# ZhangT-tech/MoCA-Video

Hardware: AMD Instinct MI355X
Metric: denoising UNet-steps/sec @16x320x512 fp16 (higher is better)
Workload: dtype f16

## Files before the change

### include/moca_hip.h

```cpp
#ifndef MOCA_HIP_H
#define MOCA_HIP_H

#include <stdint.h>

#ifdef __cplusplus
extern "C" {
#endif

#define MOCA_OK            0
#define MOCA_E_BADARG     -1
#define MOCA_E_LAUNCH     -2
#define MOCA_E_NODEVICE   -3
#define MOCA_E_GRAPH      -4

#define MOCA_A_LINEAR   0
#define MOCA_A_CONV3X3  1
#define MOCA_A_TCONV3   2

#define MOCA_EP_GEGLU   1
#define MOCA_EP_OUT_F32 2
#define MOCA_FORCE_SMALL_TILE 4
#define MOCA_EP_COLSUM 16
#define MOCA_EP_LN     32
#define MOCA_EP_GELU    8
// ... 24 lines not shown
    int32_t T;
    int32_t HW;
    int32_t flags;
    int32_t splits;
    int32_t nopad_lo;
    int32_t prefetch_kib;
    int32_t tattn_causal;
    float*      colsum;
    const float* ln_gamma;
    const float* ln_beta;
    void*       ln_out;
    int32_t     ld_ln;
    float       ln_eps;
    float*      rowsum;
    const float* lnf_part;
    const float* lnf_wsum;
    int32_t     lnf_nparts;
    int32_t     reserved2_;
    int64_t*    gstat;
    int32_t     gstat_rows;
    float       tattn_scale;
    const void* prefetch;
    int32_t     up_phase;
    int32_t     reserved4_;
    const void* a2;
    int32_t     lda2;
    int32_t     k1;
    int32_t     gstat_cpg;
    int32_t     gstat_coff;
    int32_t     wgroup_rows;
    int32_t     wgroup_stride;
} moca_gemm_params;

int moca_gemm_f16(const moca_gemm_params* p, void* stream);
int moca_gemm_colsum_rows(const moca_gemm_params* p);
int moca_gemm_ln_ok(const moca_gemm_params* p);
int moca_gemm_rowsum_cols(const moca_gemm_params* p);
int moca_gemm_lnfold_ok(const moca_gemm_params* p);
int moca_gemm_tattn_ok(const moca_gemm_params* p);
int moca_gemm_wgroup_ok(const moca_gemm_params* p);
int moca_gemm_cat_ok(const moca_gemm_params* p);
#define MOCA_ROUTE_SMALL64   1
#define MOCA_ROUTE_SMALL128  2
#define MOCA_ROUTE_GLDS128   3
#define MOCA_ROUTE_GLDS160   4
#define MOCA_ROUTE_G4        5
#define MOCA_ROUTE_W80       6
#define MOCA_ROUTE_W80W      7
#define MOCA_ROUTE_SQ256     8
#define MOCA_ROUTE_G4P       9
#define MOCA_ROUTE_SQP       10
#define MOCA_ROUTE_TATTN     11
#define MOCA_ROUTE_WS        12
int moca_gemm_route(const moca_gemm_params* p);
int moca_gemm_splitk_groupnorm_ok(const moca_gemm_params* p, int32_t HW, int32_t frames_per_stat);
int moca_gemm_splitk_groupnorm_f16(const moca_gemm_params* p, void* y, const float* gamma, const float* beta, int32_t HW,
                                   int32_t frames_per_stat, float eps, int32_t silu, int32_t write_x, void* stream);
int64_t moca_gemm_splitk_ws_bytes(int32_t M, int32_t N, int32_t splits);

int moca_groupnorm_nhwc_f16(const void* x, void* y, const float* gamma, const float* beta,
                            int32_t F, int32_t HW, int32_t C, int32_t frames_per_stat,
                            float eps, int32_t silu, float* ws, void* stream);
int64_t moca_groupnorm_ws_bytes(int32_t F, int32_t HW, int32_t C);
#define MOCA_GN_ROUTE_STREAM    1
#define MOCA_GN_ROUTE_SLAB2     2
#define MOCA_GN_ROUTE_SLAB4     3
#define MOCA_GN_ROUTE_SLAB8     4
#define MOCA_GN_ROUTE_SLABREG1  5
#define MOCA_GN_ROUTE_SLABREG2  6
#define MOCA_GN_ROUTE_SLABREG3  7
#define MOCA_GN_ROUTE_SLABREG4  8
int moca_groupnorm_route(int32_t F, int32_t HW, int32_t C, int32_t frames_per_stat);
int moca_groupnorm_nchunk(int32_t F, int32_t HW);
int moca_groupnorm_colsum_f16(const void* x, void* y, const float* gamma, const float* beta, const float* colsum,
                              int32_t tile_rows, int32_t F, int32_t HW, int32_t C, int32_t frames_per_stat,
                              float eps, int32_t silu, float* ws, void* stream);

int moca_groupnorm_fold_weights_f16(const void* w, const float* bias, const float* gamma, const float* beta, const int64_t* gstat,
                                    void* wg, float* bg, int32_t n_sg, int32_t N, int32_t K, int32_t ldw, int64_t count, float eps,
                                    void* stream);

int moca_groupnorm_gstat_f16(const void* x, void* y, const float* gamma, const float* beta, const int64_t* gstat,
                             int32_t F, int32_t HW, int32_t C, int32_t frames_per_stat,
                             float eps, int32_t silu, void* stream);
int moca_concat_channels_gstat_f16(const void* a, const void* b, void* out, int32_t F, int32_t HW, int32_t C1, int32_t C2,
                                   int32_t frames_per_stat, int64_t* gstat, void* stream);
int moca_groupnorm_gstat_cat_f16(const void* a, const void* b, void* y, const float* gamma, const float* beta,
                                 const int64_t* gstat_cat, const int64_t* gstat_b, int32_t Fb, int32_t F, int32_t HW, int32_t C1,
                                 int32_t C2, int32_t frames_per_stat, float eps, int32_t silu, void* stream);
int moca_gstat_accum_f16(const void* x, int32_t F, int32_t HW, int32_t C, int32_t frames_per_stat, int32_t cpg, int32_t coff,
                         int64_t* gstat, void* stream);
int moca_memset_zero(void* ptr, int64_t bytes, void* stream);

int moca_layernorm_f16(const void* x, void* y, const float* gamma, const float* beta,
                       int32_t M, int32_t C, float eps, void* stream);

int moca_attention_f16(const void* q, const void* k, const void* v, void* out,
                       int32_t Bq, int32_t heads, int32_t Nq, int32_t Nk,
                       int32_t ldq, int32_t ldk, int32_t ldv, int32_t ldo,
                       int32_t kv_div, float scale, void* stream);

int moca_attention_ip_f16(const void* q, const void* k, const void* v, const void* k_ip, const void* v_ip, void* out,
                          int32_t Bq, int32_t heads, int32_t Nq, int32_t Nt, int32_t Ni,
                          int32_t ldq, int32_t ldk, int32_t ldv, int32_t ldk_ip, int32_t ldv_ip, int32_t ldo,
                          int32_t kv_div, float scale, float ip_scale, void* stream);

// ... 95 lines not shown
    const int32_t* sam_idx;
    float cfg_scale, beta, one_minus_beta, gamma, one_minus_gamma;
    int32_t nW, C, Q, f, HW, wb_from;
} moca_fifo_step_params;
int moca_fifo_step_windows_f32(const moca_fifo_step_params* p, void* stream);
int moca_sam_select_masks_f32(const float* cand, const int32_t* cand_off, const int32_t* ncand, const int64_t* t_rows, float* eff,
                              int32_t* eff_idx, int32_t nW, int32_t f, int32_t HW, void* stream);
int moca_fifo_advance_f32(moca_fifo_state* state, float* queue, const float* newframe, float* emitted, int32_t n_slots,
                          int32_t emit_frame, float* mask, float* mask_sums, int32_t C, int32_t Q, int32_t HW, void* stream);
int moca_fifo_prepare_queue_f32(const float* z, const float* noise, float* queue, const float* coef_z, const float* coef_noise,
                                const int32_t* frame_idx, int32_t BC, int32_t Tz, int32_t Q, int32_t HW, void* stream);
int moca_base_set_timestep(const moca_fifo_state* state, const int64_t* table, int32_t S, int64_t* rows, int32_t n, void* stream);
int moca_base_ddim_step_f32(moca_fifo_state* state, float* x, const float* eps_c, const float* eps_u, const float* noise,
                            float* pred_x0, const float* coef, int32_t S, float cfg_scale, int32_t use_scale, int64_t n, void* stream);
#define MOCA_DDPM_X0 1
#define MOCA_DDPM_CLIP 2
#define MOCA_DDPM_SCALE 4
#define MOCA_DDPM_MASK_C0 8
int moca_ddpm_step_f32(moca_fifo_state* state, const float* x, float* out, const float* eps_c, const float* eps_u,
                       const float* noise, float* x_recon, float* mean, const float* mask, const float* x0,
                       const float* noise_q, const float* coef, const int64_t* t, int64_t t_stride, int32_t B, int32_t n_tab,
                       int64_t per, int64_t mask_inner, float cfg_scale, float temperature, int32_t flags, void* stream);
int moca_mask_frame_sums_f32(const float* mask, float* sums, int32_t frames, int32_t HW, void* stream);

int moca_freq_mix_3d_f32(const float* x, const float* noise, const float* lpf, float* out,
                         int32_t C, int32_t T, int32_t H, int32_t W, float* ws, void* stream);
int64_t moca_freq_mix_ws_bytes(int32_t C, int32_t T, int32_t H, int32_t W);
int moca_freq_filter_f32(float* lpf, int32_t T, int32_t H, int32_t W, int32_t type, int32_t n,
                         double d_s, double d_t, void* stream);

int moca_graph_begin(void* stream);
int moca_graph_end(void* stream, void** graph_exec_out);
int moca_graph_launch(void* graph_exec, void* stream);
int moca_graph_destroy(void* graph_exec);
int moca_stream_create(void** stream_out);
int moca_stream_destroy(void* stream);
int moca_stream_sync(void* stream);
int moca_event_create(void** ev_out);
int moca_event_record(void* ev, void* stream);
int moca_event_elapsed_ms(void* ev_start, void* ev_stop, float* ms_out);
int moca_event_destroy(void* ev);

#define MOCA_TUNE_GEMM_W80   0
#define MOCA_TUNE_GEMM_G4    1
#define MOCA_TUNE_GEMM_SQ256 2
#define MOCA_TUNE_GEMM_WIDE  3
#define MOCA_TUNE_GN_SLAB    4
#define MOCA_TUNE_GEMM_G4P   5
#define MOCA_TUNE_GEMM_MF32  6
#define MOCA_TUNE_GEMM_SQP   7
#define MOCA_TUNE_SQP_WALK   8
#define MOCA_TUNE_SLAB_F16   9
#define MOCA_TUNE_GEMM_WS    10
#define MOCA_TUNE_COUNT      11
int moca_set_tuning(int32_t knob, int32_t value);
int moca_debug_clock_sampler(void* buf, int32_t blocks, int32_t nsamples, const int32_t* stop, void* stream);

int moca_device_info(char* name, int32_t len, int32_t* cu_count);
const char* moca_version(void);

#ifdef __cplusplus
}
#endif
#endif
```

### moca_video_amd/csrc/gemm.hip

```cpp
#include "gemm_launch.h"

namespace {

template <int BN, int AMODE>
__global__ __launch_bounds__(256, 2) void gemm_f16_kernel(const moca_gemm_params p) {
    constexpr int NT = BN / 64;
    constexpr int B_SLOTS = BN / 32;
    constexpr int A_BYTES = BM * ROW_BYTES;
    constexpr int B_BYTES = BN * ROW_BYTES;

    extern __shared__ __attribute__((aligned(16))) char smem[];
    char* sA = smem;
    char* sB = smem + 2 * A_BYTES;

    const int tid = threadIdx.x, lane = tid & 63, wave = tid >> 6;
    const int wave_m = wave >> 1, wave_n = wave & 1;

    const int tiles_m = (p.M + BM - 1) / BM;
    const int tiles_n = p.N / BN;
    const int nblk = tiles_m * tiles_n * p.splits;
    int logical;
    remap_block<BN>(nblk, logical);
    const int split = logical % p.splits;
    const int tile = logical / p.splits;
// ... 369 lines not shown
            for (int j = 0; j < 8; ++j) { const float a = (float)v[i][j]; s += a; q += a * a; }
        }
    s = wave_sum(s); q = wave_sum(q);
    if ((tid & 63) == 0) { s_red[0][tid >> 6] = s; s_red[1][tid >> 6] = q; }
    __syncthreads();
    if (tid < cpg) {
        double a = 0.0, b = 0.0;
        for (int w = 0; w < (nthr >> 6); ++w) { a += (double)s_red[0][w]; b += (double)s_red[1][w]; }
        const double mean = a * inv_count;
        double var = b * inv_count - mean * mean;
        if (var < 0.0) var = 0.0;
        const float rstd = (float)(1.0 / sqrt(var + (double)eps));
        const float sc = rstd * gm_t;
        s_sc[tid] = sc;
        s_sh[tid] = bt_t - (float)mean * sc;
    }
    __syncthreads();
#pragma unroll
    for (int i = 0; i < CPT; ++i)
        if (mrow[i] >= 0) {
            const int c0 = ccol[i] - g * cpg;
            half8v r;
#pragma unroll
            for (int j = 0; j < 8; ++j) {
                float a = (float)v[i][j] * s_sc[c0 + j] + s_sh[c0 + j];
                if (silu) a = moca_silu(a);
                r[j] = (half_t)a;
            }
            *reinterpret_cast<half8v*>(y + (int64_t)mrow[i] * N + ccol[i]) = r;
        }
}

template <int BN, int AMODE>
int launch_gemm(const moca_gemm_params& p, hipStream_t st) {
    const int tiles_m = (p.M + BM - 1) / BM, tiles_n = p.N / BN;
    const int nblk = tiles_m * tiles_n * p.splits;
    constexpr int lds_pipe = 2 * (BM + BN) * ROW_BYTES;
    constexpr int lds_epi = BM * BN * 4;
    constexpr int lds = lds_pipe > lds_epi ? lds_pipe : lds_epi;
    if (!dyn_lds_once<&gemm_f16_kernel<BN, AMODE>>(lds)) return MOCA_E_LAUNCH;
    hipLaunchKernelGGL((gemm_f16_kernel<BN, AMODE>), dim3(nblk), dim3(256), lds, st, p);
    MOCA_CHECK_LAUNCH();
    return MOCA_OK;
}
int launch_gemm_small(int bn, const moca_gemm_params& p, hipStream_t st) {
    if (bn == 128) return with_gather(p, [&](auto am, auto) { return launch_gemm<128, decltype(am)::value>(p, st); });
    return with_gather(p, [&](auto am, auto) { return launch_gemm<64, decltype(am)::value>(p, st); });
}

enum Route : int {
    R_NONE = 0,
    R_SMALL64 = MOCA_ROUTE_SMALL64, R_SMALL128 = MOCA_ROUTE_SMALL128, R_GLDS128 = MOCA_ROUTE_GLDS128, R_GLDS160 = MOCA_ROUTE_GLDS160,
    R_G4 = MOCA_ROUTE_G4, R_W80 = MOCA_ROUTE_W80, R_W80W = MOCA_ROUTE_W80W, R_SQ256 = MOCA_ROUTE_SQ256, R_G4P = MOCA_ROUTE_G4P,
    R_SQP = MOCA_ROUTE_SQP, R_TATTN = MOCA_ROUTE_TATTN, R_WS = MOCA_ROUTE_WS,
};

void normalise_splits(moca_gemm_params& p) {
    if (p.splits < 1) p.splits = 1;
    if (p.splits > (p.K + BK - 1) / BK) p.splits = (p.K + BK - 1) / BK;
    if (p.splits > 1) {
        const int nkt = (p.K + BK - 1) / BK, kts = (nkt + p.splits - 1) / p.splits;
        p.splits = (nkt + kts - 1) / kts;
    }
}

inline int64_t a_span_bytes(const moca_gemm_params& p) {
    if (p.a_mode == MOCA_A_LINEAR) return ((int64_t)p.M * p.lda + 64) * 2;
    if (p.a_mode == MOCA_A_CONV3X3) return ((int64_t)(p.M / (p.outH * p.outW)) * p.inH * p.inW * p.C + 64) * 2;
    return ((int64_t)p.M * p.C + 64) * 2;
}
inline bool buffer_addressable(const moca_gemm_params& p) {
    if (p.a2 && ((int64_t)p.M * p.lda2 + 64) * 2 >= (1ll << 31)) return false;
    return a_span_bytes(p) < (1ll << 31) && (int64_t)p.N * p.ldw * 2 < (1ll << 31);
}

bool persistent_ok(const moca_gemm_params& p, int BN, int blocks) {
    if (p.a_mode != MOCA_A_LINEAR || p.splits != 1 || p.N % BN || p.K % 64 || !buffer_addressable(p)) return false;
    if (p.flags & ~(MOCA_EP_GEGLU | MOCA_EP_LNFOLD)) return false;
    if ((p.flags & MOCA_EP_GEGLU) && (p.residual || p.rowadd)) return false;
    return ((p.M + 255) / 256) * (p.N / BN) >= blocks;
}

Route route_of(const moca_gemm_params& p) {
    if (p.flags & MOCA_EP_TATTN) return R_TATTN;
    const int ws_mode = moca_tuning_get(MOCA_TUNE_GEMM_WS);
    if (ws_mode && moca_gemm_ws_ok(p) && (ws_mode == 2 || p.residual || p.M >= (1 << 17))) return R_WS;
    if (!p.a2 && p.wgroup_rows <= 0) {
        const int sqp_mode = moca_tuning_get(MOCA_TUNE_GEMM_SQP), g4p_mode = moca_tuning_get(MOCA_TUNE_GEMM_G4P);
        if (sqp_mode && persistent_ok(p, 256, SQP_BLOCKS) && (sqp_mode == 2 || (p.flags & MOCA_EP_GEGLU))) return R_SQP;
        if (g4p_mode && persistent_ok(p, 128, G4P_BLOCKS) && (g4p_mode == 2 || (p.flags & MOCA_EP_GEGLU))) return R_G4P;
    }
    const int w80_mode = moca_tuning_get(MOCA_TUNE_GEMM_W80);
    const int tiles320 = ((p.M + 319) / 320) * (p.N / 160);
    if (w80_mode && p.N % 160 == 0 && !(p.flags & (MOCA_EP_GEGLU | MOCA_EP_OUT_F32 | MOCA_FORCE_SMALL_TILE)) && p.M > 160 &&
        (tiles320 * p.splits >= 200 || w80_mode == 2) && fast_gather(p) && buffer_addressable(p)) {
        if (p.flags & MOCA_EP_LN) return R_W80W;
        const int wide_mode = moca_tuning_get(MOCA_TUNE_GEMM_WIDE);
        if (wide_mode == 0 || p.N % 320) return R_W80;
        return (p.a_mode == MOCA_A_LINEAR || wide_mode == 2) ? R_W80W : R_W80;
    }
    const int g4_mode = moca_tuning_get(MOCA_TUNE_GEMM_G4);
    const bool use_g4 = !(p.flags & MOCA_EP_OUT_F32) &&
                        (g4_mode == 2 || (g4_mode == 1 && (p.flags & MOCA_EP_GEGLU) && p.K <= 640 && p.M < (1 << 17)));
    const int sq256_mode = moca_tuning_get(MOCA_TUNE_GEMM_SQ256);
    if (sq256_mode && p.a_mode == MOCA_A_LINEAR && p.N % 256 == 0 && p.N >= 2560 && p.M >= 512 && fast_gather(p) && buffer_addressable(p) &&
        !(p.flags & (MOCA_EP_OUT_F32 | MOCA_FORCE_SMALL_TILE)) && ((p.M + 255) / 256) * (p.N / 256) * p.splits >= 200 &&
        (sq256_mode == 2 || !use_g4)) return R_SQ256;
    const int big_bn = (p.N % 128 == 0) ? 128 : (p.N % 160 == 0 ? 160 : 0);
    if (big_bn != 0 && p.M > 128 && !(p.flags & MOCA_FORCE_SMALL_TILE)) {
        if (big_bn == 128) return use_g4 ? R_G4 : R_GLDS128;
        return R_GLDS160;
    }
    return p.N % 128 == 0 ? R_SMALL128 : R_SMALL64;
}

constexpr int CAN_SPLITK = 1 << 16, CAN_A2 = 1 << 17, CAN_WGROUP = 1 << 18, CAN_UP_PHASE = 1 << 19;
constexpr int EP_STATS = MOCA_EP_COLSUM | MOCA_EP_GSTAT;
struct RouteInfo { int tm, tn, can; };
RouteInfo route_info(Route r) {
    constexpr int GLDS = MOCA_EP_GEGLU | MOCA_EP_OUT_F32 | EP_STATS | MOCA_EP_ROWSUM | MOCA_EP_LNFOLD | CAN_SPLITK | CAN_UP_PHASE;
    constexpr int W80 = EP_STATS | MOCA_EP_ROWSUM | MOCA_EP_LNFOLD | CAN_SPLITK | CAN_UP_PHASE | CAN_A2 | CAN_WGROUP;
    switch (r) {
        case R_SMALL64: return {BM, 64, MOCA_EP_OUT_F32 | MOCA_EP_GELU | CAN_SPLITK};
        case R_SMALL128: return {BM, 128, MOCA_EP_GEGLU | MOCA_EP_OUT_F32 | MOCA_EP_GELU | CAN_SPLITK};
        case R_GLDS128: return {256, 128, GLDS};
        case R_GLDS160: return {256, 160, GLDS};
        case R_G4: return {256, 128, MOCA_EP_GEGLU | MOCA_EP_LNFOLD | CAN_SPLITK | CAN_UP_PHASE};
        case R_W80: return {320, 160, W80};
        case R_W80W: return {160, 320, W80 | MOCA_EP_LN};
        case R_SQ256: return {256, 256, MOCA_EP_GEGLU | MOCA_EP_LNFOLD | CAN_SPLITK};
        case R_G4P: return {256, 128, MOCA_EP_GEGLU | MOCA_EP_LNFOLD};
        case R_SQP: return {256, 256, MOCA_EP_GEGLU | MOCA_EP_LNFOLD};
        case R_TATTN: return {320, 192, MOCA_EP_TATTN | MOCA_EP_LNFOLD};
        case R_WS: return {32, 80, MOCA_EP_ROWSUM | MOCA_EP_GSTAT | CAN_WGROUP};
        case R_NONE: break;
    }
    return {0, 0, 0};
}

bool route_can(Route r, const moca_gemm_params& p) {
    const RouteInfo ri = route_info(r);
    const int f = p.flags & ~(MOCA_FORCE_SMALL_TILE | MOCA_EP_SLABS);
    const int wants = f | (p.splits > 1 ? CAN_SPLITK : 0) | (p.a2 ? CAN_A2 : 0) | (p.wgroup_rows ? CAN_WGROUP : 0) | (p.up_phase ? CAN_UP_PHASE : 0);
    if (r == R_NONE || (wants & ~ri.can) || p.wgroup_rows < 0) return false;
    if (r == R_WS) return true;
    const bool linear1 = p.a_mode == MOCA_A_LINEAR && p.splits == 1;
    if (r == R_TATTN) {
        if (!linear1 || !fast_gather(p) || !buffer_addressable(p) || p.residual || p.rowadd || (p.flags & MOCA_FORCE_SMALL_TILE)) return false;
        if (p.N % 192 || p.T != 16 || p.HW <= 0 || p.HW % 20 || p.M % (16 * p.HW)) return false;
        if (p.ldo % 4 || p.ldo < p.N / 3) return false;
        return p.tattn_causal == 0 || (p.tattn_causal == 1 && p.tattn_scale > 0.f);
    }
    if ((f & EP_STATS) && (p.splits != 1 || (f & (MOCA_EP_GEGLU | MOCA_EP_OUT_F32)))) return false;
    if ((f & MOCA_EP_ROWSUM) && (p.splits != 1 || (f & (MOCA_EP_GEGLU | MOCA_EP_OUT_F32 | EP_STATS | MOCA_EP_LN | MOCA_EP_GELU)))) return false;
    if ((f & MOCA_EP_LN) && !(linear1 && p.N == 320 && !(f & EP_STATS))) return false;
    if ((f & MOCA_EP_LNFOLD) && !(linear1 && !(f & (MOCA_EP_OUT_F32 | EP_STATS | MOCA_EP_LN | MOCA_EP_ROWSUM | MOCA_EP_GELU)) &&
                                  !((r == R_GLDS128 || r == R_GLDS160) && (f & MOCA_EP_GEGLU)))) return false;
    if ((f & MOCA_EP_GELU) && (f & MOCA_EP_GEGLU)) return false;
    if (p.a2) {
        if (!linear1 || (f & ~(EP_STATS | MOCA_EP_ROWSUM))) return false;
        if (p.k1 <= 0 || p.k1 >= p.K || p.k1 % 64 || (p.K - p.k1) % 64 || p.lda % 8 || p.lda2 % 8 || p.lda < p.k1 || p.lda2 < p.K - p.k1) return false;
    }
    if (p.wgroup_rows) {
        if (!linear1 || p.a2 || p.wgroup_stride < p.N * p.ldw || (f & ~(EP_STATS | MOCA_EP_ROWSUM | MOCA_EP_LN))) return false;
        if (p.M % p.wgroup_rows || p.wgroup_rows % ri.tm) return false;
        if ((int64_t)(p.M / p.wgroup_rows) * p.wgroup_stride * 2 >= (1ll << 31)) return false;
    }
    if (p.up_phase && (p.splits != 1 || p.M <= 160 || !fast_gather(p) || p.residual || p.rowadd || (f & ~MOCA_EP_GSTAT) ||
                       (p.N % 128 && p.N % 160))) return false;
    return true;
}

Route checked_route(const moca_gemm_params& p) {
    const Route r = route_of(p);
    return route_can(r, p) ? r : R_NONE;
}

Route query_route(const moca_gemm_params* pp, int flag, moca_gemm_params& p) {
    if (!pp) return R_NONE;
    p = *pp;
    if (p.M <= 0 || p.N <= 0 || p.K <= 0 || p.N % 64 || p.K % 8) return R_NONE;
// ... 25 lines not shown
    if (p.splits > 1 && !p.splitk_ws) return R_NONE;
    if (p.prefetch_kib < 0 || (p.prefetch_kib > 0 && (!p.prefetch || (reinterpret_cast<uintptr_t>(p.prefetch) & 15)))) return R_NONE;
    if ((p.flags & MOCA_EP_GELU) && (p.splits != 1 || !((p.flags & MOCA_FORCE_SMALL_TILE) || p.M <= 128))) return R_NONE;
    normalise_splits(p);
    if ((p.flags & MOCA_EP_SLABS) && (p.splits < 2 || (p.flags & ~MOCA_EP_SLABS))) return R_NONE;
    if (p.up_phase && p.a_mode != MOCA_A_CONV3X3) return R_NONE;
    switch (p.a_mode) {
        case MOCA_A_LINEAR:
            if (!p.a2 && (p.lda % 8 || p.lda < p.K)) return R_NONE;
            break;
        case MOCA_A_CONV3X3:
            if (p.up_phase < 0 || p.up_phase > 4) return R_NONE;
            if (p.C % 8 || p.K != (p.up_phase ? 4 : 9) * p.C || p.inH <= 0 || p.inW <= 0 || p.outH <= 0 || p.outW <= 0) return R_NONE;
            if (p.up_phase && (p.stride != 1 || p.up || p.nopad_lo)) return R_NONE;
            if (p.stride != 1 && p.stride != 2) return R_NONE;
            if (p.nopad_lo != 0 && (p.nopad_lo != 1 || p.stride != 2 || p.up || (p.inH | p.inW) & 1)) return R_NONE;
            if (p.up && (p.stride != 1 || p.outH != 2 * p.inH || p.outW != 2 * p.inW)) return R_NONE;
            if (!p.up && p.stride == 1 && (p.outH != p.inH || p.outW != p.inW)) return R_NONE;
            if (p.stride == 2 && (p.outH != (p.inH - 1) / 2 + 1 || p.outW != (p.inW - 1) / 2 + 1)) return R_NONE;
            if (p.M % (p.outH * p.outW)) return R_NONE;
            break;
        case MOCA_A_TCONV3:
            if (p.C % 8 || p.K != 3 * p.C || p.T <= 0 || p.HW <= 0 || p.M % (p.T * p.HW)) return R_NONE;
            break;
        default:
            return R_NONE;
    }
    if (p.a2 && p.a_mode != MOCA_A_LINEAR) return R_NONE;
    if (p.gstat_cpg < 0 || p.gstat_coff < 0 || ((p.gstat_cpg || p.gstat_coff) && !(p.flags & MOCA_EP_GSTAT))) return R_NONE;
    if (p.tattn_causal && !(p.flags & MOCA_EP_TATTN)) return R_NONE;
    const Route r = checked_route(p);
    if (r == R_NONE) return R_NONE;
    if ((p.flags & MOCA_EP_COLSUM) && !p.colsum) return R_NONE;
    if ((p.flags & MOCA_EP_LN) && !(p.ln_gamma && p.ln_beta && p.ln_out && p.ld_ln % 8 == 0)) return R_NONE;
    if ((p.flags & MOCA_EP_ROWSUM) && !p.rowsum) return R_NONE;
    if ((p.flags & MOCA_EP_LNFOLD) && !(p.lnf_part && p.lnf_wsum && p.lnf_nparts >= 1)) return R_NONE;
    if ((p.flags & MOCA_EP_GSTAT) &&
        !(p.gstat && !(p.flags & MOCA_EP_COLSUM) && p.gstat_rows > 0 && p.gstat_rows % route_info(r).tm == 0 && p.M % p.gstat_rows == 0 &&
          (p.gstat_cpg > 0 ? (p.gstat_coff + p.N - 1) / p.gstat_cpg < 32 : (p.N % 32 == 0 && p.gstat_coff == 0)))) return R_NONE;
    p.reserved4_ = 0;
    if ((int64_t)p.M * (geglu ? p.N / 2 : p.N) * 2 >= (128ll << 20)) p.reserved4_ |= 1;
    if (slab_f16(r, p)) p.reserved4_ |= 4;
    return r;
}

int launch_route(Route r, const moca_gemm_params& p, hipStream_t st) {
    switch (r) {
        case R_TATTN: return moca_gemm_w80s_launch(3, p, st);
        case R_WS: return moca_gemm_ws_launch(p, st);
        case R_SQP: return moca_gemm_sqp_launch(p, st);
        case R_G4P: return moca_gemm_g4p_launch(p, st);
        case R_W80: return moca_gemm_w80s_launch(0, p, st);
        case R_W80W: return moca_gemm_w80s_launch(1, p, st);
        case R_SQ256: return moca_gemm_w80s_launch(2, p, st);
        case R_G4: return moca_gemm_g4_launch(p, st);
        case R_GLDS128: return moca_gemm_glds_launch(128, p, st);
        case R_GLDS160: return moca_gemm_glds_launch(160, p, st);
        case R_SMALL128: return launch_gemm_small(128, p, st);
        case R_SMALL64: return launch_gemm_small(64, p, st);
        case R_NONE: break;
    }
    return MOCA_E_BADARG;
}

}

#ifdef MOCA_STAMPS
extern "C" int moca_debug_stamps(unsigned long long* host_out, int n_blocks) {
    if (n_blocks > STAMP_BLOCKS) n_blocks = STAMP_BLOCKS;
    return hipMemcpyFromSymbol(host_out, HIP_SYMBOL(g_stamps), (size_t)n_blocks * STAMP_SLOTS * 8) == hipSuccess ? 0 : -2;
}
#endif

extern "C" int moca_gemm_route(const moca_gemm_params* pp) {
    moca_gemm_params p;
    return prepare(pp, p);
}

extern "C" int moca_gemm_colsum_rows(const moca_gemm_params* pp) {
    moca_gemm_params p;
    return route_info(query_route(pp, (pp && (pp->flags & MOCA_EP_GSTAT)) ? 0 : MOCA_EP_COLSUM, p)).tm;
}
extern "C" int moca_gemm_rowsum_cols(const moca_gemm_params* pp) {
    moca_gemm_params p;
    return route_info(query_route(pp, MOCA_EP_ROWSUM, p)).tn;
}
extern "C" int moca_gemm_ln_ok(const moca_gemm_params* pp) {
    moca_gemm_params p;
    return query_route(pp, MOCA_EP_LN, p) != R_NONE;
}
extern "C" int moca_gemm_lnfold_ok(const moca_gemm_params* pp) {
    moca_gemm_params p;
    return query_route(pp, MOCA_EP_LNFOLD, p) != R_NONE;
}
extern "C" int moca_gemm_tattn_ok(const moca_gemm_params* pp) {
    moca_gemm_params p;
    return query_route(pp, MOCA_EP_TATTN, p) != R_NONE;
}
extern "C" int moca_gemm_cat_ok(const moca_gemm_params* pp) {
    moca_gemm_params p;
    return query_route(pp, 0, p) != R_NONE && p.a2;
}
extern "C" int moca_gemm_wgroup_ok(const moca_gemm_params* pp) {
    moca_gemm_params p;
    return query_route(pp, 0, p) != R_NONE && p.wgroup_rows > 0;
}
// ... 58 lines not shown
```

### moca_video_amd/csrc/gemm_diag.hip

```cpp
#ifndef MOCA_DIAG_NAME
#error "gemm_diag.hip is the unit of the diagnostic builds: compile it with -DMOCA_DIAG_NAME"
#endif
#include "gemm.hip"
#include "gemm_tiled.hip"
#include "gemm_persistent.hip"
```

### moca_video_amd/csrc/gemm_launch.h

```cpp
#ifndef MOCA_GEMM_LAUNCH_H
#define MOCA_GEMM_LAUNCH_H
#include "gemm_device.h"

int moca_gemm_glds_launch(int bn, const moca_gemm_params& p, hipStream_t st);
int moca_gemm_g4_launch(const moca_gemm_params& p, hipStream_t st);
int moca_gemm_w80s_launch(int shape, const moca_gemm_params& p, hipStream_t st);
int moca_gemm_g4p_launch(const moca_gemm_params& p, hipStream_t st);
int moca_gemm_sqp_launch(const moca_gemm_params& p, hipStream_t st);

namespace {

constexpr int G4P_BLOCKS = 512;
constexpr int SQP_BLOCKS = 256;

static int choose_xcd_n(const moca_gemm_params& p, int tiles_m, int tiles_n, int BN) {
    if (p.splits != 1 || p.a_mode != MOCA_A_LINEAR) return 1;
    const double Wtot = (double)p.N * p.K * 2, Atot = (double)p.M * p.K * 2;
    auto cost = [&](int xn) {
        const int xm = 8 / xn;
        const double wsub = (double)(tiles_n / xn) * BN * p.K * 2;
        return (wsub <= 3.6e6 ? xm * Wtot : tiles_m * Wtot) + xn * Atot;
    };
    double best = cost(1);
    int best_xn = 1;
    for (int xn = 2; xn <= 8; xn *= 2) {
        if (tiles_m % (8 / xn) || tiles_n % xn) continue;
        const double c = cost(xn);
        if (c < 0.8 * best) { best = c; best_xn = xn; }
    }
    return best_xn;
}

inline bool fast_gather(const moca_gemm_params& p) {
    return (p.a_mode == MOCA_A_LINEAR) ? (p.K % BK == 0 && p.K <= 8192) : (p.C % BK == 0 && p.C <= 8192);
}
template <typename F>
int with_gather(const moca_gemm_params& p, F f) {
    const bool fast = fast_gather(p);
    if (p.a_mode == MOCA_A_LINEAR) return fast ? f(int_c<MOCA_A_LINEAR>{}, yes_t{}) : f(int_c<MOCA_A_LINEAR>{}, no_t{});
    if (p.a_mode == MOCA_A_CONV3X3) return fast ? f(int_c<MOCA_A_CONV3X3>{}, yes_t{}) : f(int_c<MOCA_A_CONV3X3>{}, no_t{});
    return fast ? f(int_c<MOCA_A_TCONV3>{}, yes_t{}) : f(int_c<MOCA_A_TCONV3>{}, no_t{});
}

template <auto KERNEL>
bool dyn_lds_once(int lds) {
    static bool attr_set = false;
    if (!attr_set) {
        if (hipFuncSetAttribute(reinterpret_cast<const void*>(KERNEL), hipFuncAttributeMaxDynamicSharedMemorySize, lds) != hipSuccess) return false;
        attr_set = true;
    }
    return true;
}

}

#endif
```

### moca_video_amd/csrc/runtime.hip

```cpp
#include "common.h"
#include <string.h>
#include <stdio.h>
#include <stdlib.h>

extern "C" int moca_graph_begin(void* stream) {
    if (hipStreamBeginCapture(moca_stream(stream), hipStreamCaptureModeThreadLocal) != hipSuccess) return MOCA_E_GRAPH;
    return MOCA_OK;
}

extern "C" int moca_graph_end(void* stream, void** graph_exec_out) {
    if (!graph_exec_out) return MOCA_E_BADARG;
    hipGraph_t g = nullptr;
    if (hipStreamEndCapture(moca_stream(stream), &g) != hipSuccess || !g) return MOCA_E_GRAPH;
    hipGraphExec_t ge = nullptr;
    hipError_t e = hipGraphInstantiate(&ge, g, nullptr, nullptr, 0);
    (void)hipGraphDestroy(g);
    if (e != hipSuccess || !ge) return MOCA_E_GRAPH;
    *graph_exec_out = reinterpret_cast<void*>(ge);
    return MOCA_OK;
}

extern "C" int moca_graph_launch(void* graph_exec, void* stream) {
    if (!graph_exec) return MOCA_E_BADARG;
    if (hipGraphLaunch(reinterpret_cast<hipGraphExec_t>(graph_exec), moca_stream(stream)) != hipSuccess) return MOCA_E_GRAPH;
// ... 45 lines not shown
    int dev = 0;
    if (hipGetDevice(&dev) != hipSuccess) return MOCA_E_NODEVICE;
    hipDeviceProp_t prop;
    if (hipGetDeviceProperties(&prop, dev) != hipSuccess) return MOCA_E_NODEVICE;
    if (name && len > 0) {
        strncpy(name, prop.gcnArchName, (size_t)len - 1);
        name[len - 1] = 0;
    }
    if (cu_count) *cu_count = prop.multiProcessorCount;
    return MOCA_OK;
}

__global__ __launch_bounds__(256) void zero_kernel(uint4* __restrict__ p, int64_t n16, unsigned char* __restrict__ tail, int ntail) {
    for (int64_t i = (int64_t)blockIdx.x * 256 + threadIdx.x; i < n16; i += (int64_t)gridDim.x * 256) p[i] = uint4{0u, 0u, 0u, 0u};
    if (blockIdx.x == 0 && (int)threadIdx.x < ntail) tail[threadIdx.x] = 0;
}

extern "C" int moca_memset_zero(void* ptr, int64_t bytes, void* stream) {
    if (!ptr || bytes < 0 || (reinterpret_cast<uintptr_t>(ptr) & 15)) return MOCA_E_BADARG;
    if (bytes == 0) return MOCA_OK;
    const int64_t n16 = bytes / 16;
    int blocks = (int)((n16 + 255) / 256);
    if (blocks < 1) blocks = 1;
    if (blocks > 1024) blocks = 1024;
    hipLaunchKernelGGL(zero_kernel, dim3(blocks), dim3(256), 0, moca_stream(stream), reinterpret_cast<uint4*>(ptr), n16,
                       reinterpret_cast<unsigned char*>(ptr) + n16 * 16, (int)(bytes - n16 * 16));
    MOCA_CHECK_LAUNCH();
    return MOCA_OK;
}

__global__ __launch_bounds__(64) void clock_sampler_kernel(unsigned long long* __restrict__ buf, int nsamples, const volatile int* stop) {
#if defined(__HIP_DEVICE_COMPILE__)
    if (threadIdx.x) return;
    unsigned long long* b = buf + (size_t)blockIdx.x * nsamples * 2;
    for (int i = 0; i < nsamples; ++i) {
        unsigned long long t, r;
        asm volatile("s_memtime %0\n\ts_memrealtime %1\n\ts_waitcnt lgkmcnt(0)" : "=s"(t), "=s"(r)::"memory");
        b[2 * i] = t;
        b[2 * i + 1] = r;
        if (stop && *stop) break;
        __builtin_amdgcn_s_sleep(127);
        __builtin_amdgcn_s_sleep(127);
    }
#endif
}
extern "C" int moca_debug_clock_sampler(void* buf, int32_t blocks, int32_t nsamples, const int32_t* stop, void* stream) {
    if (!buf || blocks < 1 || blocks > 64 || nsamples < 1 || nsamples > (1 << 20)) return MOCA_E_BADARG;
    hipLaunchKernelGGL(clock_sampler_kernel, dim3(blocks), dim3(64), 0, moca_stream(stream), reinterpret_cast<unsigned long long*>(buf), nsamples,
                       reinterpret_cast<const volatile int*>(stop));
    MOCA_CHECK_LAUNCH();
    return MOCA_OK;
}

static int g_tuning[MOCA_TUNE_COUNT] = {1, 1, 1, 1, 1, 1, 0, 1, 0, 0, 1};
int moca_tuning_get(int knob) { return (knob >= 0 && knob < MOCA_TUNE_COUNT) ? g_tuning[knob] : 0; }
extern "C" int moca_set_tuning(int32_t knob, int32_t value) {
    if (knob < 0 || knob >= MOCA_TUNE_COUNT || value < 0 || value > 2) return MOCA_E_BADARG;
    const int old = g_tuning[knob];
    g_tuning[knob] = value;
    return old;
}
```

### moca_video_amd/lib.py

```python
from __future__ import annotations

import ctypes as C
import os

import torch

_HERE = os.path.dirname(os.path.abspath(__file__))
LIB_PATH = os.environ.get("MOCA_HIP_LIB") or os.path.join(_HERE, "libmoca_hip.so")

MOCA_A_LINEAR, MOCA_A_CONV3X3, MOCA_A_TCONV3 = 0, 1, 2
MOCA_EP_GEGLU, MOCA_EP_OUT_F32, MOCA_FORCE_SMALL_TILE, MOCA_EP_GELU, MOCA_EP_COLSUM, MOCA_EP_LN = 1, 2, 4, 8, 16, 32
MOCA_EP_ROWSUM, MOCA_EP_LNFOLD, MOCA_EP_GSTAT, MOCA_EP_TATTN, MOCA_EP_SLABS = 64, 128, 256, 512, 1024
MOCA_TUNE_GEMM_W80, MOCA_TUNE_GEMM_G4, MOCA_TUNE_GEMM_SQ256, MOCA_TUNE_GEMM_WIDE, MOCA_TUNE_GN_SLAB, MOCA_TUNE_GEMM_G4P, MOCA_TUNE_GEMM_MF32, MOCA_TUNE_GEMM_SQP, MOCA_TUNE_SQP_WALK = 0, 1, 2, 3, 4, 5, 6, 7, 8
MOCA_TUNE_SLAB_F16 = 9
MOCA_TUNE_GEMM_WS = 10
MOCA_DDPM_X0, MOCA_DDPM_CLIP, MOCA_DDPM_SCALE, MOCA_DDPM_MASK_C0 = 1, 2, 4, 8
(MOCA_ROUTE_SMALL64, MOCA_ROUTE_SMALL128, MOCA_ROUTE_GLDS128, MOCA_ROUTE_GLDS160, MOCA_ROUTE_G4, MOCA_ROUTE_W80, MOCA_ROUTE_W80W,
 MOCA_ROUTE_SQ256, MOCA_ROUTE_G4P, MOCA_ROUTE_SQP, MOCA_ROUTE_TATTN, MOCA_ROUTE_WS) = range(1, 13)
(MOCA_GN_ROUTE_STREAM, MOCA_GN_ROUTE_SLAB2, MOCA_GN_ROUTE_SLAB4, MOCA_GN_ROUTE_SLAB8, MOCA_GN_ROUTE_SLABREG1, MOCA_GN_ROUTE_SLABREG2,
 MOCA_GN_ROUTE_SLABREG3, MOCA_GN_ROUTE_SLABREG4) = range(1, 9)

_ERR = {0: "ok", -1: "bad argument (shape/alignment contract)", -2: "HIP launch/runtime error",
        -3: "no gfx950 device", -4: "graph capture/replay failed"}


class MocaHipError(RuntimeError):
    pass


class GemmParams(C.Structure):
    _fields_ = [
        ("a", C.c_void_p), ("w", C.c_void_p), ("out", C.c_void_p), ("bias", C.c_void_p),
        ("rowadd", C.c_void_p), ("residual", C.c_void_p), ("splitk_ws", C.c_void_p),
        ("M", C.c_int32), ("N", C.c_int32), ("K", C.c_int32),
        ("lda", C.c_int32), ("ldw", C.c_int32), ("ldo", C.c_int32), ("ldr", C.c_int32), ("ld_rowadd", C.c_int32),
        ("rowadd_div", C.c_int32), ("a_mode", C.c_int32), ("C", C.c_int32),
        ("inH", C.c_int32), ("inW", C.c_int32), ("outH", C.c_int32), ("outW", C.c_int32),
        ("stride", C.c_int32), ("up", C.c_int32), ("T", C.c_int32), ("HW", C.c_int32),
        ("flags", C.c_int32), ("splits", C.c_int32), ("nopad_lo", C.c_int32), ("prefetch_kib", C.c_int32),
        ("tattn_causal", C.c_int32),
        ("colsum", C.c_void_p), ("ln_gamma", C.c_void_p), ("ln_beta", C.c_void_p), ("ln_out", C.c_void_p),
        ("ld_ln", C.c_int32), ("ln_eps", C.c_float),
        ("rowsum", C.c_void_p), ("lnf_part", C.c_void_p), ("lnf_wsum", C.c_void_p),
        ("lnf_nparts", C.c_int32), ("reserved2_", C.c_int32),
        ("gstat", C.c_void_p), ("gstat_rows", C.c_int32), ("tattn_scale", C.c_float),
        ("prefetch", C.c_void_p), ("up_phase", C.c_int32), ("reserved4_", C.c_int32),
        ("a2", C.c_void_p), ("lda2", C.c_int32), ("k1", C.c_int32), ("gstat_cpg", C.c_int32), ("gstat_coff", C.c_int32),
        ("wgroup_rows", C.c_int32), ("wgroup_stride", C.c_int32),
    ]


class FifoState(C.Structure):
    _fields_ = [("head", C.c_int32), ("iter", C.c_int32), ("seed_lo", C.c_uint32), ("seed_hi", C.c_uint32),
                ("ext_noise", C.c_int32), ("reserved_", C.c_int32 * 3)]


class FifoStepParams(C.Structure):
    _fields_ = [
        ("state", C.c_void_p), ("x", C.c_void_p), ("eps_c", C.c_void_p), ("eps_u", C.c_void_p), ("noise", C.c_void_p),
        ("momentum", C.c_void_p), ("queue", C.c_void_p), ("x_prev", C.c_void_p), ("pred_x0", C.c_void_p), ("coef", C.c_void_p),
        ("win_start", C.c_void_p), ("mask", C.c_void_p), ("mask_sums", C.c_void_p), ("mask_frame", C.c_void_p),
        ("enh", C.c_void_p), ("cond", C.c_void_p), ("sam_eff", C.c_void_p), ("sam_idx", C.c_void_p),
        ("cfg_scale", C.c_float), ("beta", C.c_float), ("one_minus_beta", C.c_float), ("gamma", C.c_float),
        ("one_minus_gamma", C.c_float),
        ("nW", C.c_int32), ("C", C.c_int32), ("Q", C.c_int32), ("f", C.c_int32), ("HW", C.c_int32), ("wb_from", C.c_int32),
    ]


_vp, _i32, _i64, _f32, _f64 = C.c_void_p, C.c_int32, C.c_int64, C.c_float, C.c_double
SIGNATURES = {
    "moca_gemm_f16": (C.c_int, [C.POINTER(GemmParams), _vp]),
# ... 137 lines not shown
```

Baseline: 60.36.

## Add halo-tiled 3x3 conv implicit GEMM kernel reusing input rows across taps

Adds a new W80H route for stride-1 3x3 convolutions with input width 64 or 32. The kernel loads a halo slab of input rows into LDS once per channel slice and reuses it across all nine taps, instead of gathering A separately per tap. It streams weights through a ring buffer with a 512-thread schedule, and is on by default via a new tuning knob. The intent is to cut global and LDS traffic for the A operand in the conv GEMMs, at the cost of a complex hand-scheduled pipeline with more LDS usage.

```diff
diff --git a/include/moca_hip.h b/include/moca_hip.h
--- a/include/moca_hip.h
+++ b/include/moca_hip.h
@@ -100,6 +100,7 @@
 #define MOCA_ROUTE_SQP       10
 #define MOCA_ROUTE_TATTN     11
 #define MOCA_ROUTE_WS        12
+#define MOCA_ROUTE_W80H      13
 int moca_gemm_route(const moca_gemm_params* p);
 int moca_gemm_splitk_groupnorm_ok(const moca_gemm_params* p, int32_t HW, int32_t frames_per_stat);
 int moca_gemm_splitk_groupnorm_f16(const moca_gemm_params* p, void* y, const float* gamma, const float* beta, int32_t HW,
@@ -301,7 +302,8 @@
 #define MOCA_TUNE_SQP_WALK   8
 #define MOCA_TUNE_SLAB_F16   9
 #define MOCA_TUNE_GEMM_WS    10
-#define MOCA_TUNE_COUNT      11
+#define MOCA_TUNE_CONV_HALO  11
+#define MOCA_TUNE_COUNT      12
 int moca_set_tuning(int32_t knob, int32_t value);
 int moca_debug_clock_sampler(void* buf, int32_t blocks, int32_t nsamples, const int32_t* stop, void* stream);
 
diff --git a/moca_video_amd/csrc/gemm.hip b/moca_video_amd/csrc/gemm.hip
--- a/moca_video_amd/csrc/gemm.hip
+++ b/moca_video_amd/csrc/gemm.hip
@@ -445,7 +445,7 @@
     R_NONE = 0,
     R_SMALL64 = MOCA_ROUTE_SMALL64, R_SMALL128 = MOCA_ROUTE_SMALL128, R_GLDS128 = MOCA_ROUTE_GLDS128, R_GLDS160 = MOCA_ROUTE_GLDS160,
     R_G4 = MOCA_ROUTE_G4, R_W80 = MOCA_ROUTE_W80, R_W80W = MOCA_ROUTE_W80W, R_SQ256 = MOCA_ROUTE_SQ256, R_G4P = MOCA_ROUTE_G4P,
-    R_SQP = MOCA_ROUTE_SQP, R_TATTN = MOCA_ROUTE_TATTN, R_WS = MOCA_ROUTE_WS,
+    R_SQP = MOCA_ROUTE_SQP, R_TATTN = MOCA_ROUTE_TATTN, R_WS = MOCA_ROUTE_WS, R_W80H = MOCA_ROUTE_W80H,
 };
 
 void normalise_splits(moca_gemm_params& p) {
@@ -472,6 +472,12 @@
     if (p.flags & ~(MOCA_EP_GEGLU | MOCA_EP_LNFOLD)) return false;
     if ((p.flags & MOCA_EP_GEGLU) && (p.residual || p.rowadd)) return false;
     return ((p.M + 255) / 256) * (p.N / BN) >= blocks;
+}
+
+bool halo_ok(const moca_gemm_params& p) {
+    if (p.a_mode != MOCA_A_CONV3X3 || p.stride != 1 || p.up || p.up_phase || p.nopad_lo || p.splits != 1 || p.a2 || p.wgroup_rows) return false;
+    if ((p.inW != 64 && p.inW != 32) || p.inH % (320 / p.inW) || p.C % 32 || p.C > 8192) return false;
+    return !(p.flags & ~(MOCA_EP_COLSUM | MOCA_EP_GSTAT | MOCA_EP_ROWSUM));
 }
 
 Route route_of(const moca_gemm_params& p) {
@@ -485,8 +491,10 @@
     }
     const int w80_mode = moca_tuning_get(MOCA_TUNE_GEMM_W80);
     const int tiles320 = ((p.M + 319) / 320) * (p.N / 160);
+    const bool halo = moca_tuning_get(MOCA_TUNE_CONV_HALO) && halo_ok(p);
     if (w80_mode && p.N % 160 == 0 && !(p.flags & (MOCA_EP_GEGLU | MOCA_EP_OUT_F32 | MOCA_FORCE_SMALL_TILE)) && p.M > 160 &&
-        (tiles320 * p.splits >= 200 || w80_mode == 2) && fast_gather(p) && buffer_addressable(p)) {
+        (tiles320 * p.splits >= 200 || w80_mode == 2) && (fast_gather(p) || halo) && buffer_addressable(p)) {
+        if (halo) return R_W80H;
         if (p.flags & MOCA_EP_LN) return R_W80W;
         const int wide_mode = moca_tuning_get(MOCA_TUNE_GEMM_WIDE);
         if (wide_mode == 0 || p.N % 320) return R_W80;
@@ -520,6 +528,7 @@
         case R_GLDS160: return {256, 160, GLDS};
         case R_G4: return {256, 128, MOCA_EP_GEGLU | MOCA_EP_LNFOLD | CAN_SPLITK | CAN_UP_PHASE};
         case R_W80: return {320, 160, W80};
+        case R_W80H: return {320, 160, EP_STATS | MOCA_EP_ROWSUM};
         case R_W80W: return {160, 320, W80 | MOCA_EP_LN};
         case R_SQ256: return {256, 256, MOCA_EP_GEGLU | MOCA_EP_LNFOLD | CAN_SPLITK};
         case R_G4P: return {256, 128, MOCA_EP_GEGLU | MOCA_EP_LNFOLD};
@@ -651,6 +660,7 @@
         case R_G4P: return moca_gemm_g4p_launch(p, st);
         case R_W80: return moca_gemm_w80s_launch(0, p, st);
         case R_W80W: return moca_gemm_w80s_launch(1, p, st);
+        case R_W80H: return moca_gemm_w80h_launch(p, st);
         case R_SQ256: return moca_gemm_w80s_launch(2, p, st);
         case R_G4: return moca_gemm_g4_launch(p, st);
         case R_GLDS128: return moca_gemm_glds_launch(128, p, st);
diff --git a/moca_video_amd/csrc/gemm_diag.hip b/moca_video_amd/csrc/gemm_diag.hip
--- a/moca_video_amd/csrc/gemm_diag.hip
+++ b/moca_video_amd/csrc/gemm_diag.hip
@@ -4,3 +4,4 @@
 #include "gemm.hip"
 #include "gemm_tiled.hip"
 #include "gemm_persistent.hip"
+#include "gemm_halo.hip"
diff --git a/moca_video_amd/csrc/gemm_halo.hip b/moca_video_amd/csrc/gemm_halo.hip
--- /dev/null
+++ b/moca_video_amd/csrc/gemm_halo.hip
@@ -0,0 +1,203 @@
+#include "gemm_launch.h"
+
+namespace {
+
+template <int IW>
+__global__ __launch_bounds__(512, 2) void gemm_w80h_kernel(const moca_gemm_params p) {
+#if defined(__HIP_DEVICE_COMPILE__)
+    constexpr int MT = 5, NT = 5, KS = 32, RB = 64;
+    constexpr int TM = 320, BN = 160, WTN = 80;
+    constexpr int NB = IW / 16;
+    constexpr int HR = TM / IW + 2;
+    constexpr int ROWB = IW * RB + 64;
+    constexpr int HSLOT = 64 + HR * ROWB;
+    constexpr int NP2 = 2 * HR * NB;
+    constexpr int WT = BN * RB;
+    constexpr int WRING = 4 * HSLOT, DUMP = WRING + 4 * WT;
+    constexpr int APER = 12;
+    static_assert(8 * APER >= NP2 && HSLOT + (MT + 1) * ROWB < 65536, "halo schedule / ds_read immediates");
+
+    extern __shared__ __attribute__((aligned(16))) char smem[];
+
+    const int tid = threadIdx.x, lane = tid & 63;
+    const int wave = __builtin_amdgcn_readfirstlane(tid >> 6);
+    const int wave_m = wave >> 1, wave_n = wave & 1, wq = wave & 3;
+    const int cb = wave_m % NB, rg = wave_m / NB;
+    const bool late = wave >= 4;
+    const int half = late ? 1 : 0;
+
+    const int tiles_n = p.N / BN;
+    const int nblk = (p.M / TM) * tiles_n;
+    if (prefetch_block(p, nblk, 512)) return;
+    int logical;
+    remap_block<BN>(nblk, logical);
+    const int tile_m = logical / tiles_n, tile_n = logical % tiles_n;
+    const int m0 = tile_m * TM, n0 = tile_n * BN;
+    const int hw = p.inH * IW;
+    const int frame = m0 / hw;
+    const int y0 = (m0 - frame * hw) / IW;
+    const int pix0 = frame * hw;
+    const int npairs = (p.C / KS + 1) >> 1;
+
+    if (tid < 16 * (HR + 1)) {
+        const int sl = tid / (4 * (HR + 1)), rem = tid - sl * 4 * (HR + 1);
+        *reinterpret_cast<f32x4*>(smem + sl * HSLOT + (rem >> 2) * ROWB + (rem & 3) * 16) = f32x4{0.f, 0.f, 0.f, 0.f};
+    }
+
+    const __amdgpu_buffer_rsrc_t rsrc_a = __builtin_amdgcn_make_buffer_rsrc(const_cast<void*>(p.a), 0, OOB_OFF, 0x00020000);
+    const __amdgpu_buffer_rsrc_t rsrc_w = __builtin_amdgcn_make_buffer_rsrc(const_cast<void*>(p.w), 0, OOB_OFF, 0x00020000);
+    const unsigned a_voff = (unsigned)(((lane & 15) * p.C + (lane >> 4) * 8) * 2);
+    const int lrow = lane >> 2, pch = lane & 3;
+    const int lch = pch ^ ((0x78 >> (2 * ((lrow >> 2) & 3))) & 3);
+    unsigned w_off[3];
+#pragma unroll
+    for (int g = 0; g < 3; ++g) w_off[g] = (unsigned)(((int64_t)(n0 + ((g < 2 ? g * 4 + wq : 8 + (wq & 1))) * 16 + lrow) * p.ldw + lch * 8) * 2);
+
+    auto dma_a = [&](int idx, int jpA, bool live, int y0v, int pix0v) {
+        const int par = idx & 1, pq = idx >> 1;
+        const int Y = pq / NB, q = pq % NB;
+        const int iy = y0v - 1 + Y, slice = 2 * jpA + par;
+        const bool listed = live && idx < NP2;
+        const bool ok = listed && iy >= 0 && iy < p.inH && slice * KS < p.C;
+        const unsigned soff = ok ? ((unsigned)((pix0v + iy * IW + q * 16) * p.C + slice * KS)) * 2u : 0u;
+        const int dst = listed ? ((jpA & 1) * 2 + par) * HSLOT + 64 + Y * ROWB + q * 1024 : DUMP;
+        __builtin_amdgcn_raw_ptr_buffer_load_lds(rsrc_a, (lds_ptr)smem + dst, 16, ok ? a_voff : OOB_OFF, soff, 0, 0);
+    };
+    auto issue = [&](int t2, int jp2, int wsl, int tA, int jpA, int y0v, int pix0v, int wavev) {
+        const bool wok = jp2 < npairs && (!late || (2 * jp2 + 1) * KS < p.C);
+        const unsigned w_s = wok ? (unsigned)((t2 * p.C + jp2 * 64 + half * KS) * 2) : 0u;
+        const lds_ptr wd = (lds_ptr)smem + WRING + (wsl + half) * WT;
+        const bool alive = tA < 8 && jpA < npairs;
+        __builtin_amdgcn_raw_ptr_buffer_load_lds(rsrc_w, wd + wq * 1024, 16, wok ? w_off[0] : OOB_OFF, w_s, 0, 0);
+        __builtin_amdgcn_raw_ptr_buffer_load_lds(rsrc_w, wd + (4 + wq) * 1024, 16, wok ? w_off[1] : OOB_OFF, w_s, 0, 0);
+        if (wq < 2) __builtin_amdgcn_raw_ptr_buffer_load_lds(rsrc_w, wd + (8 + wq) * 1024, 16, wok ? w_off[2] : OOB_OFF, w_s, 0, 0);
+        else dma_a(tA * APER + half * 2 + (wq - 2), jpA, alive, y0v, pix0v);
+        dma_a(tA * APER + 4 + wavev, jpA, alive, y0v, pix0v);
+    };
+
+    const int fr = lane & 15, fg = lane >> 4;
+    f32x4 acc[MT][NT];
+#pragma unroll
+    for (int nt = 0; nt < NT; ++nt) {
+        f32x4 bv = {0.f, 0.f, 0.f, 0.f};
+        if (p.bias) bv = *reinterpret_cast<const f32x4*>(p.bias + n0 + wave_n * WTN + nt * 16 + 4 * fg);
+#pragma unroll
+        for (int mt = 0; mt < MT; ++mt) acc[mt][nt] = bv;
+    }
+
+    const int swz = (fg ^ ((0x78 >> (2 * ((fr >> 2) & 3))) & 3)) << 4;
+    const int b_off0 = WRING + (wave_n * WTN + fr) * RB + swz;
+    int a_base[3], a_cur[3];
+#pragma unroll
+    for (int dx = 0; dx < 3; ++dx) {
+        const int X = fr + dx - 1;
+        int o = cb * 1024 + (X >> 4) * 1024 + (X & 15) * 16 + fg * 256;
+        if (X < 0 && cb == 0) o = -16;
+        if (X > 15 && cb == NB - 1) o = IW * RB;
+        a_base[dx] = 64 + rg * 5 * ROWB + o;
+    }
+
+    half8v af[2][MT], bf[2][NT];
+
+#pragma unroll
+    for (int k = 0; k < (NP2 + 7) / 8; ++k) dma_a(k * 8 + wave, 0, true, y0, pix0);
+    issue(0, 0, 0, 8, 0, y0, pix0, wave);
+    issue(1, 0, 2, 8, 0, y0, pix0, wave);
+    asm volatile("s_waitcnt vmcnt(4) lgkmcnt(0)" ::: "memory");
+    __builtin_amdgcn_s_barrier();
+    if (late) __builtin_amdgcn_s_barrier();
+
+    int wsl = 0;
+    for (int jp = 0; jp < npairs; ++jp) {
+#pragma unroll
+        for (int dx = 0; dx < 3; ++dx) a_cur[dx] = a_base[dx] + (jp & 1) * 2 * HSLOT;
+        auto iter = [&](auto tap_tag) {
+            constexpr int T = decltype(tap_tag)::value, DY = T / 3, DX = T % 3;
+            const char* we = smem + wsl * WT + b_off0;
+            const char* ae = smem + a_cur[DX];
+#pragma unroll
+            for (int r = 0; r < NT; ++r) bf[0][r] = *reinterpret_cast<const half8v*>(we + r * 1024);
+#pragma unroll
+            for (int r = 0; r < MT; ++r) af[0][r] = *reinterpret_cast<const half8v*>(ae + (r + DY) * ROWB);
+            asm volatile("s_waitcnt lgkmcnt(0)" ::: "memory");
+            __builtin_amdgcn_sched_barrier(0);
+            __builtin_amdgcn_s_barrier();
+            __builtin_amdgcn_s_setprio(1);
+#pragma unroll
+            for (int j = 0; j < MT * NT; ++j) {
+                const int mt = j / NT, nt = j % NT;
+                acc[mt][nt] = __builtin_amdgcn_mfma_f32_16x16x32_f16(bf[0][nt], af[0][mt], acc[mt][nt], 0, 0, 0);
+                if (j % 2 == 0 && j / 2 < MT + NT) {
+                    const int r = j / 2;
+                    __builtin_amdgcn_sched_barrier(0);
+                    if (r < NT) bf[1][r] = *reinterpret_cast<const half8v*>(we + WT + r * 1024);
+                    else af[1][r - NT] = *reinterpret_cast<const half8v*>(ae + HSLOT + (r - NT + DY) * ROWB);
+                    __builtin_amdgcn_sched_barrier(0);
+                }
+            }
+            __builtin_amdgcn_s_setprio(0);
+            asm volatile("s_waitcnt lgkmcnt(0)" ::: "memory");
+            __builtin_amdgcn_sched_barrier(0);
+            __builtin_amdgcn_s_barrier();
+            int y0v = y0, pix0v = pix0, wavev = wave;
+            asm volatile("" : "+s"(y0v), "+s"(pix0v), "+s"(wavev));
+            issue((T + 2) % 9, jp + (T + 2) / 9, wsl, T, jp + 1, y0v, pix0v, wavev);
+            asm volatile("s_waitcnt vmcnt(4)" ::: "memory");
+            __builtin_amdgcn_sched_barrier(0);
+            __builtin_amdgcn_s_barrier();
+            __builtin_amdgcn_s_setprio(1);
+#pragma unroll
+            for (int mt = 0; mt < MT; ++mt)
+#pragma unroll
+                for (int nt = 0; nt < NT; ++nt)
+                    acc[mt][nt] = __builtin_amdgcn_mfma_f32_16x16x32_f16(bf[1][nt], af[1][mt], acc[mt][nt], 0, 0, 0);
+            __builtin_amdgcn_s_setprio(0);
+            __builtin_amdgcn_sched_barrier(0);
+            __builtin_amdgcn_s_barrier();
+            wsl ^= 2;
+        };
+        iter(int_c<0>{}); iter(int_c<1>{}); iter(int_c<2>{});
+        iter(int_c<3>{}); iter(int_c<4>{}); iter(int_c<5>{});
+        iter(int_c<6>{}); iter(int_c<7>{}); iter(int_c<8>{});
+    }
+    if (!late) __builtin_amdgcn_s_barrier();
+    asm volatile("s_waitcnt vmcnt(0) lgkmcnt(0)" ::: "memory");
+    __builtin_amdgcn_s_barrier();
+
+    constexpr int pitch = BN * 2 + 16;
+#pragma unroll
+    for (int nt = 0; nt < NT; ++nt) {
+        const int col = wave_n * WTN + nt * 16 + 4 * fg;
+#pragma unroll
+        for (int mt = 0; mt < MT; ++mt) {
+            const int row = (rg * 5 + mt) * IW + cb * 16 + fr;
+            *reinterpret_cast<half4v*>(smem + row * pitch + col * 2) = __builtin_convertvector(acc[mt][nt], half4v);
+        }
+    }
+    __syncthreads();
+    if (p.flags & (MOCA_EP_COLSUM | MOCA_EP_GSTAT)) store_fp16_tile_colsum<TM, BN>(p, smem, reinterpret_cast<float*>(smem + TM * pitch), pitch, m0, n0, tile_m, tid);
+    else if (p.flags & MOCA_EP_ROWSUM) store_fp16_tile_rowsum<512, BN, 4>(p, smem, pitch, TM, m0, n0, tid);
+    else store_fp16_tile<512>(p, smem, pitch, TM, BN, m0, n0, tid);
+#endif
+}
+
+template <int IW>
+int launch_gemm_w80h(const moca_gemm_params& p, hipStream_t st) {
+    constexpr int HR = 320 / IW + 2;
+    constexpr int lds = 4 * (64 + HR * (IW * 64 + 64)) + 4 * 160 * 64 + 1024;
+    const int nblk = (p.M / 320) * (p.N / 160);
+    moca_gemm_params pl = p;
+    pl.reserved4_ = (pl.reserved4_ & 0xff) | (1 << 8);
+    if (!dyn_lds_once<&gemm_w80h_kernel<IW>>(lds)) return MOCA_E_LAUNCH;
+    hipLaunchKernelGGL(gemm_w80h_kernel<IW>, dim3(nblk + prefetch_blocks(pl)), dim3(512), lds, st, pl);
+    MOCA_CHECK_LAUNCH();
+    return MOCA_OK;
+}
+
+}
+
+int moca_gemm_w80h_launch(const moca_gemm_params& p, hipStream_t st) {
+    if (p.inW == 64) return launch_gemm_w80h<64>(p, st);
+    if (p.inW == 32) return launch_gemm_w80h<32>(p, st);
+    return MOCA_E_BADARG;
+}
diff --git a/moca_video_amd/csrc/gemm_launch.h b/moca_video_amd/csrc/gemm_launch.h
--- a/moca_video_amd/csrc/gemm_launch.h
+++ b/moca_video_amd/csrc/gemm_launch.h
@@ -5,6 +5,7 @@
 int moca_gemm_glds_launch(int bn, const moca_gemm_params& p, hipStream_t st);
 int moca_gemm_g4_launch(const moca_gemm_params& p, hipStream_t st);
 int moca_gemm_w80s_launch(int shape, const moca_gemm_params& p, hipStream_t st);
+int moca_gemm_w80h_launch(const moca_gemm_params& p, hipStream_t st);
 int moca_gemm_g4p_launch(const moca_gemm_params& p, hipStream_t st);
 int moca_gemm_sqp_launch(const moca_gemm_params& p, hipStream_t st);
 
diff --git a/moca_video_amd/csrc/runtime.hip b/moca_video_amd/csrc/runtime.hip
--- a/moca_video_amd/csrc/runtime.hip
+++ b/moca_video_amd/csrc/runtime.hip
@@ -121,7 +121,7 @@
     return MOCA_OK;
 }
 
-static int g_tuning[MOCA_TUNE_COUNT] = {1, 1, 1, 1, 1, 1, 0, 1, 0, 0, 1};
+static int g_tuning[MOCA_TUNE_COUNT] = {1, 1, 1, 1, 1, 1, 0, 1, 0, 0, 1, 1};
 int moca_tuning_get(int knob) { return (knob >= 0 && knob < MOCA_TUNE_COUNT) ? g_tuning[knob] : 0; }
 extern "C" int moca_set_tuning(int32_t knob, int32_t value) {
     if (knob < 0 || knob >= MOCA_TUNE_COUNT || value < 0 || value > 2) return MOCA_E_BADARG;
diff --git a/moca_video_amd/lib.py b/moca_video_amd/lib.py
--- a/moca_video_amd/lib.py
+++ b/moca_video_amd/lib.py
@@ -14,9 +14,10 @@
 MOCA_TUNE_GEMM_W80, MOCA_TUNE_GEMM_G4, MOCA_TUNE_GEMM_SQ256, MOCA_TUNE_GEMM_WIDE, MOCA_TUNE_GN_SLAB, MOCA_TUNE_GEMM_G4P, MOCA_TUNE_GEMM_MF32, MOCA_TUNE_GEMM_SQP, MOCA_TUNE_SQP_WALK = 0, 1, 2, 3, 4, 5, 6, 7, 8
 MOCA_TUNE_SLAB_F16 = 9
 MOCA_TUNE_GEMM_WS = 10
+MOCA_TUNE_CONV_HALO = 11
 MOCA_DDPM_X0, MOCA_DDPM_CLIP, MOCA_DDPM_SCALE, MOCA_DDPM_MASK_C0 = 1, 2, 4, 8
 (MOCA_ROUTE_SMALL64, MOCA_ROUTE_SMALL128, MOCA_ROUTE_GLDS128, MOCA_ROUTE_GLDS160, MOCA_ROUTE_G4, MOCA_ROUTE_W80, MOCA_ROUTE_W80W,
- MOCA_ROUTE_SQ256, MOCA_ROUTE_G4P, MOCA_ROUTE_SQP, MOCA_ROUTE_TATTN, MOCA_ROUTE_WS) = range(1, 13)
+ MOCA_ROUTE_SQ256, MOCA_ROUTE_G4P, MOCA_ROUTE_SQP, MOCA_ROUTE_TATTN, MOCA_ROUTE_WS, MOCA_ROUTE_W80H) = range(1, 14)
 (MOCA_GN_ROUTE_STREAM, MOCA_GN_ROUTE_SLAB2, MOCA_GN_ROUTE_SLAB4, MOCA_GN_ROUTE_SLAB8, MOCA_GN_ROUTE_SLABREG1, MOCA_GN_ROUTE_SLABREG2,
  MOCA_GN_ROUTE_SLABREG3, MOCA_GN_ROUTE_SLABREG4) = range(1, 9)
 
```

After: 61.01, median of 6. 1.01x the previous value.
